# facebookresearch/multimodal

Measured on NVIDIA H100. Metric: image-text pairs/sec (CLIP ViT-B/16 contrastive pretrain step, bs=512/GPU), higher is better.
Workload: dtype bf16

## Files before the change

multimodal_b200/csrc/common.cuh:

```cuda
#pragma once
#include <cuda.h>
#include <cuda_bf16.h>
#include <cuda_runtime.h>
#include <stdint.h>
#include <stdio.h>

namespace mmb {

__device__ __forceinline__ uint32_t smem_u32(const void* p) {
  return static_cast<uint32_t>(__cvta_generic_to_shared(p));
}

__device__ __forceinline__ uint64_t global_timer_ns() {
  uint64_t t;
  asm volatile("mov.u64 %0, %%globaltimer;" : "=l"(t));
  return t;
}

#ifndef MMB_WATCHDOG_NS
#define MMB_WATCHDOG_NS 4000000000ull
#endif

__device__ __forceinline__ void mbar_init(uint64_t* bar, uint32_t count) {
  asm volatile("mbarrier.init.shared::cta.b64 [%0], %1;" ::"r"(smem_u32(bar)), "r"(count) : "memory");
}
__device__ __forceinline__ void fence_mbar_init() {
  asm volatile("fence.mbarrier_init.release.cluster;" ::: "memory");
}
__device__ __forceinline__ void fence_proxy_async_smem() {
  asm volatile("fence.proxy.async.shared::cta;" ::: "memory");
}
__device__ __forceinline__ void mbar_arrive_expect_tx(uint64_t* bar, uint32_t bytes) {
  asm volatile("mbarrier.arrive.expect_tx.shared::cta.b64 _, [%0], %1;" ::"r"(smem_u32(bar)), "r"(bytes)
               : "memory");
}
__device__ __forceinline__ void mbar_arrive(uint64_t* bar) {
  asm volatile("mbarrier.arrive.shared::cta.b64 _, [%0];" ::"r"(smem_u32(bar)) : "memory");
}
__device__ __forceinline__ void mbar_arrive_cluster(uint64_t* bar, uint32_t cta) {
  uint32_t remote;
  asm volatile("mapa.shared::cluster.u32 %0, %1, %2;" : "=r"(remote) : "r"(smem_u32(bar)), "r"(cta));
  asm volatile("mbarrier.arrive.shared::cluster.b64 _, [%0];" ::"r"(remote) : "memory");
}
__device__ __forceinline__ bool mbar_try_wait(uint64_t* bar, uint32_t parity) {
  uint32_t ok;
  asm volatile(
      "{\n\t.reg .pred p;\n\t"
      "mbarrier.try_wait.parity.shared::cta.b64 p, [%1], %2;\n\t"
      "selp.u32 %0, 1, 0, p;\n\t}"
      : "=r"(ok)
      : "r"(smem_u32(bar)), "r"(parity)
      : "memory");
  return ok != 0;
}
__device__ __forceinline__ void mbar_wait(uint64_t* bar, uint32_t parity) {
  if (mbar_try_wait(bar, parity)) return;
  uint32_t polls = 0;
  uint64_t t0 = 0;
  while (!mbar_try_wait(bar, parity)) {
#ifdef MMB_WAIT_NANOSLEEP
    __nanosleep(MMB_WAIT_NANOSLEEP);
#endif
    if ((++polls & 1023u) == 0) {
      const uint64_t now = global_timer_ns();
      if (t0 == 0) t0 = now;
      else if (now - t0 > MMB_WATCHDOG_NS) {
        printf("mmb watchdog: mbarrier wait timed out (block %d thread %d parity %u)\n", (int)blockIdx.x,
               (int)threadIdx.x, parity);
        __trap();
      }
    }
  }
}

__device__ __forceinline__ void mbar_wait_quiet(uint64_t* bar, uint32_t parity) {
  if (mbar_try_wait(bar, parity)) return;
  uint32_t polls = 0;
  uint64_t t0 = 0;
  while (!mbar_try_wait(bar, parity)) {
    if ((++polls & 1023u) == 0) {
      const uint64_t now = global_timer_ns();
      if (t0 == 0) t0 = now;
      else if (now - t0 > MMB_WATCHDOG_NS) __trap();
    }
  }
}

__device__ __forceinline__ void tma_prefetch_desc(const CUtensorMap* m) {
  asm volatile("prefetch.tensormap [%0];" ::"l"(reinterpret_cast<uint64_t>(m)) : "memory");
}
__device__ __forceinline__ void tma_prefetch_l2_2d(const CUtensorMap* m, int c0, int c1) {
  asm volatile("cp.async.bulk.prefetch.tensor.2d.L2.global.tile [%0, {%1, %2}];" ::"l"(reinterpret_cast<uint64_t>(m)),
               "r"(c0), "r"(c1)
               : "memory");
}
__device__ __forceinline__ void tma_load_2d(const CUtensorMap* m, uint64_t* bar, void* smem, int c0, int c1) {
  asm volatile(
      "cp.async.bulk.tensor.2d.shared::cluster.global.mbarrier::complete_tx::bytes [%0], [%1, {%3, %4}], [%2];"
      ::"r"(smem_u32(smem)), "l"(reinterpret_cast<uint64_t>(m)), "r"(smem_u32(bar)), "r"(c0), "r"(c1)
      : "memory");
}
__device__ __forceinline__ void tma_load_3d(const CUtensorMap* m, uint64_t* bar, void* smem, int c0, int c1,
                                            int c2) {
  asm volatile(
      "cp.async.bulk.tensor.3d.shared::cluster.global.mbarrier::complete_tx::bytes [%0], [%1, {%3, %4, %5}], [%2];"
      ::"r"(smem_u32(smem)), "l"(reinterpret_cast<uint64_t>(m)), "r"(smem_u32(bar)), "r"(c0), "r"(c1), "r"(c2)
      : "memory");
}
__device__ __forceinline__ void tma_store_2d(const CUtensorMap* m, const void* smem, int c0, int c1) {
  asm volatile("cp.async.bulk.tensor.2d.global.shared::cta.bulk_group [%0, {%2, %3}], [%1];" ::"l"(
                   reinterpret_cast<uint64_t>(m)),
               "r"(smem_u32(smem)), "r"(c0), "r"(c1)
               : "memory");
}
__device__ __forceinline__ void tma_store_3d(const CUtensorMap* m, const void* smem, int c0, int c1, int c2) {
  asm volatile("cp.async.bulk.tensor.3d.global.shared::cta.bulk_group [%0, {%2, %3, %4}], [%1];" ::"l"(
                   reinterpret_cast<uint64_t>(m)),
               "r"(smem_u32(smem)), "r"(c0), "r"(c1), "r"(c2)
               : "memory");
}
__device__ __forceinline__ void tma_reduce_add_2d(const CUtensorMap* m, const void* smem, int c0, int c1) {
  asm volatile("cp.reduce.async.bulk.tensor.2d.global.shared::cta.add.bulk_group [%0, {%2, %3}], [%1];" ::"l"(
                   reinterpret_cast<uint64_t>(m)),
               "r"(smem_u32(smem)), "r"(c0), "r"(c1)
               : "memory");
}
__device__ __forceinline__ void tma_store_commit() { asm volatile("cp.async.bulk.commit_group;" ::: "memory"); }
template <int N>
__device__ __forceinline__ void tma_store_wait_read() {
  asm volatile("cp.async.bulk.wait_group.read %0;" ::"n"(N) : "memory");
}
template <int N>
__device__ __forceinline__ void tma_store_wait_all() {
  asm volatile("cp.async.bulk.wait_group %0;" ::"n"(N) : "memory");
}

__device__ __forceinline__ uint32_t cluster_ctarank() {
  uint32_t r;
  asm volatile("mov.u32 %0, %%cluster_ctarank;" : "=r"(r));
  return r;
}
__device__ __forceinline__ void cluster_sync_all() {
  asm volatile("barrier.cluster.arrive.release.aligned;\n\tbarrier.cluster.wait.acquire.aligned;" ::: "memory");
}
__device__ __forceinline__ void tma_load_2d_multicast(const CUtensorMap* m, uint64_t* bar, void* smem, int c0, int c1,
                                                      uint16_t cta_mask) {
  asm volatile(
      "cp.async.bulk.tensor.2d.shared::cluster.global.mbarrier::complete_tx::bytes.multicast::cluster [%0], [%1, {%3, "
      "%4}], [%2], %5;" ::"r"(smem_u32(smem)),
      "l"(reinterpret_cast<uint64_t>(m)), "r"(smem_u32(bar)), "r"(c0), "r"(c1), "h"(cta_mask)
      : "memory");
}

__device__ __forceinline__ uint64_t make_smem_desc_sw128(uint32_t saddr, uint32_t lbo_bytes, uint32_t sbo_bytes) {
  uint64_t d = 0;
  d |= (uint64_t)((saddr & 0x3FFFFu) >> 4);
  d |= (uint64_t)((lbo_bytes >> 4) & 0x3FFFu) << 16;
  d |= (uint64_t)((sbo_bytes >> 4) & 0x3FFFu) << 32;
  d |= (uint64_t)1 << 62;
  return d;
}
__device__ __forceinline__ void wgmma_fence() { asm volatile("wgmma.fence.sync.aligned;" ::: "memory"); }
__device__ __forceinline__ void wgmma_commit() { asm volatile("wgmma.commit_group.sync.aligned;" ::: "memory"); }
template <int N>
__device__ __forceinline__ void wgmma_wait() {
  asm volatile("wgmma.wait_group.sync.aligned %0;" ::"n"(N) : "memory");
}
template <int TA, int TB>
__device__ __forceinline__ void wgmma_m64n256k16(float (&d)[128], uint64_t adesc, uint64_t bdesc, uint32_t accumulate) {
  asm volatile(
      "{\n\t.reg .pred p;\n\t"
      "setp.ne.b32 p, %130, 0;\n\t"
      "wgmma.mma_async.sync.aligned.m64n256k16.f32.bf16.bf16 "
      "{"
      "%0, %1, %2, %3, %4, %5, %6, %7, %8, %9, %10, %11, %12, %13, %14, %15, "
      "%16, %17, %18, %19, %20, %21, %22, %23, %24, %25, %26, %27, %28, %29, %30, %31, "
      "%32, %33, %34, %35, %36, %37, %38, %39, %40, %41, %42, %43, %44, %45, %46, %47, "
      "%48, %49, %50, %51, %52, %53, %54, %55, %56, %57, %58, %59, %60, %61, %62, %63, "
      "%64, %65, %66, %67, %68, %69, %70, %71, %72, %73, %74, %75, %76, %77, %78, %79, "
      "%80, %81, %82, %83, %84, %85, %86, %87, %88, %89, %90, %91, %92, %93, %94, %95, "
      "%96, %97, %98, %99, %100, %101, %102, %103, %104, %105, %106, %107, %108, %109, %110, %111, "
      "%112, %113, %114, %115, %116, %117, %118, %119, %120, %121, %122, %123, %124, %125, %126, %127"
      "}, %128, %129, p, 1, 1, %131, %132;\n\t}"
      : "+f"(d[0]), "+f"(d[1]), "+f"(d[2]), "+f"(d[3]), "+f"(d[4]), "+f"(d[5]), "+f"(d[6]), "+f"(d[7]),
        "+f"(d[8]), "+f"(d[9]), "+f"(d[10]), "+f"(d[11]), "+f"(d[12]), "+f"(d[13]), "+f"(d[14]), "+f"(d[15]),
        "+f"(d[16]), "+f"(d[17]), "+f"(d[18]), "+f"(d[19]), "+f"(d[20]), "+f"(d[21]), "+f"(d[22]), "+f"(d[23]),
        "+f"(d[24]), "+f"(d[25]), "+f"(d[26]), "+f"(d[27]), "+f"(d[28]), "+f"(d[29]), "+f"(d[30]), "+f"(d[31]),
        "+f"(d[32]), "+f"(d[33]), "+f"(d[34]), "+f"(d[35]), "+f"(d[36]), "+f"(d[37]), "+f"(d[38]), "+f"(d[39]),
        "+f"(d[40]), "+f"(d[41]), "+f"(d[42]), "+f"(d[43]), "+f"(d[44]), "+f"(d[45]), "+f"(d[46]), "+f"(d[47]),
        "+f"(d[48]), "+f"(d[49]), "+f"(d[50]), "+f"(d[51]), "+f"(d[52]), "+f"(d[53]), "+f"(d[54]), "+f"(d[55]),
        "+f"(d[56]), "+f"(d[57]), "+f"(d[58]), "+f"(d[59]), "+f"(d[60]), "+f"(d[61]), "+f"(d[62]), "+f"(d[63]),
        "+f"(d[64]), "+f"(d[65]), "+f"(d[66]), "+f"(d[67]), "+f"(d[68]), "+f"(d[69]), "+f"(d[70]), "+f"(d[71]),
        "+f"(d[72]), "+f"(d[73]), "+f"(d[74]), "+f"(d[75]), "+f"(d[76]), "+f"(d[77]), "+f"(d[78]), "+f"(d[79]),
        "+f"(d[80]), "+f"(d[81]), "+f"(d[82]), "+f"(d[83]), "+f"(d[84]), "+f"(d[85]), "+f"(d[86]), "+f"(d[87]),
        "+f"(d[88]), "+f"(d[89]), "+f"(d[90]), "+f"(d[91]), "+f"(d[92]), "+f"(d[93]), "+f"(d[94]), "+f"(d[95]),
        "+f"(d[96]), "+f"(d[97]), "+f"(d[98]), "+f"(d[99]), "+f"(d[100]), "+f"(d[101]), "+f"(d[102]), "+f"(d[103]),
        "+f"(d[104]), "+f"(d[105]), "+f"(d[106]), "+f"(d[107]), "+f"(d[108]), "+f"(d[109]), "+f"(d[110]), "+f"(d[111]),
        "+f"(d[112]), "+f"(d[113]), "+f"(d[114]), "+f"(d[115]), "+f"(d[116]), "+f"(d[117]), "+f"(d[118]), "+f"(d[119]),
        "+f"(d[120]), "+f"(d[121]), "+f"(d[122]), "+f"(d[123]), "+f"(d[124]), "+f"(d[125]), "+f"(d[126]), "+f"(d[127])
      : "l"(adesc), "l"(bdesc), "r"(accumulate), "n"(TA), "n"(TB));
}

template <int N>
__device__ __forceinline__ void setmaxnreg_dec() { asm volatile("setmaxnreg.dec.sync.aligned.u32 %0;" ::"n"(N)); }
template <int N>
__device__ __forceinline__ void setmaxnreg_inc() { asm volatile("setmaxnreg.inc.sync.aligned.u32 %0;" ::"n"(N)); }

__device__ __forceinline__ void ldsm_x4(uint32_t (&r)[4], uint32_t addr) {
  asm volatile("ldmatrix.sync.aligned.m8n8.x4.shared.b16 {%0,%1,%2,%3}, [%4];"
               : "=r"(r[0]), "=r"(r[1]), "=r"(r[2]), "=r"(r[3])
               : "r"(addr));
}
__device__ __forceinline__ void ldsm_x4_t(uint32_t (&r)[4], uint32_t addr) {
  asm volatile("ldmatrix.sync.aligned.m8n8.x4.trans.shared.b16 {%0,%1,%2,%3}, [%4];"
               : "=r"(r[0]), "=r"(r[1]), "=r"(r[2]), "=r"(r[3])
               : "r"(addr));
}
__device__ __forceinline__ void mma16816(float (&d)[4], const uint32_t (&a)[4], uint32_t b0, uint32_t b1) {
  asm volatile(
      "mma.sync.aligned.m16n8k16.row.col.f32.bf16.bf16.f32 {%0,%1,%2,%3}, {%4,%5,%6,%7}, {%8,%9}, {%0,%1,%2,%3};"
      : "+f"(d[0]), "+f"(d[1]), "+f"(d[2]), "+f"(d[3])
      : "r"(a[0]), "r"(a[1]), "r"(a[2]), "r"(a[3]), "r"(b0), "r"(b1));
}

__device__ __forceinline__ uint32_t pack_bf16x2(float lo, float hi) {
  __nv_bfloat162 v = __floats2bfloat162_rn(lo, hi);
  return *reinterpret_cast<uint32_t*>(&v);
}
__device__ __forceinline__ float bf16_lo(uint32_t v) { return __uint_as_float(v << 16); }
__device__ __forceinline__ float bf16_hi(uint32_t v) { return __uint_as_float(v & 0xFFFF0000u); }

__device__ __forceinline__ float ex2_approx(float x) {
  float y;
  asm("ex2.approx.ftz.f32 %0, %1;" : "=f"(y) : "f"(x));
  return y;
}
__device__ __forceinline__ float rcp_approx(float x) {
  float y;
  asm("rcp.approx.ftz.f32 %0, %1;" : "=f"(y) : "f"(x));
  return y;
}
__device__ __forceinline__ float fast_sigmoid(float z) {
  return rcp_approx(1.f + ex2_approx(-1.4426950408889634f * z));
}
__device__ __forceinline__ float tanh_approx(float x) {
  float y;
  asm("tanh.approx.f32 %0, %1;" : "=f"(y) : "f"(x));
  return y;
}
__device__ __forceinline__ float quick_gelu(float x) {
  const float t = tanh_approx(0.851f * x), h = 0.5f * x;
  return fmaf(h, t, h);
}
__device__ __forceinline__ float quick_gelu_grad(float x) {
  const float u = 0.851f * x;
  const float t = tanh_approx(u);
  return fmaf(0.5f, fmaf(u, fmaf(-t, t, 1.f), t), 0.5f);
}
__device__ __forceinline__ float gelu_erf(float x) { return 0.5f * x * (1.f + erff(x * 0.70710678118654752f)); }
__device__ __forceinline__ float gelu_erf_grad(float x) {
  return 0.5f * (1.f + erff(x * 0.70710678118654752f)) + x * 0.3989422804014327f * ex2_approx(-0.7213475204444817f * x * x);
}
template <int ACT>
__device__ __forceinline__ float act_fn(float x) { return ACT == 0 ? quick_gelu(x) : gelu_erf(x); }
template <int ACT>
__device__ __forceinline__ float act_grad(float x) { return ACT == 0 ? quick_gelu_grad(x) : gelu_erf_grad(x); }

}
```

multimodal_b200/csrc/gemm.cu:

```cuda
#include "common.cuh"
#include "mmb200_internal.h"
#include <stdlib.h>
#include <mutex>

namespace mmb {

constexpr int BLOCK_M = 128;
constexpr int BLOCK_N = 256;
constexpr int BLOCK_K = 64;
constexpr int WG_K = 16;
constexpr int STAGES = 4;
constexpr int A_BYTES = BLOCK_M * BLOCK_K * 2;
constexpr int B_BYTES = BLOCK_N * BLOCK_K * 2;
constexpr int GEMM_THREADS = 384;
constexpr int STG_BYTES = 64 * 128;
constexpr int EPI_SMEM = 4 * STG_BYTES;
constexpr int GEMM_SMEM_BYTES = 1024  + STAGES * (A_BYTES + B_BYTES) + EPI_SMEM + 256 ;
static_assert(GEMM_SMEM_BYTES <= 227 * 1024, "H100: at most 227 KB of shared memory per block");

struct GemmArgs {
  int M, N, K;
  int m_tiles, n_tiles, splits, kb_total, kb_per_split;
  float alpha;
  const float* bias;
  const __nv_bfloat16* aux;
  long long ld_aux;
  void* d0; void* d1;
  long long ldd0, ldd1;
  float* colsum_part;
  float* splitk_ws;
  int ws_rows;
  int accumulate;
  int f32_direct;
  const float* ce_log_scale;
  int ce_label0;
  const int* ce_labels;
  int ce_n_total;
  float ce_smoothing;
  float ce_gs;
  float ce_loss_weight;
  const float* ce_lse_row;
  const float* ce_row_w;
  const float* ce_lse_col;
  const float* ce_col_w;
  int ce_col_lo, ce_col_hi;
  float4* ce_part;
  int ce_part_ld, ce_part0;
  float* ce_xlabel;
};

__device__ __forceinline__ void wg_bar_sync(int cw) { asm volatile("bar.sync %0, 128;" ::"r"(2 + cw) : "memory"); }

template <bool A_MN, bool B_MN, int EPI, int ACT, bool CLU>
__global__ void __launch_bounds__(GEMM_THREADS, 1)
gemm_kernel(const __grid_constant__ CUtensorMap tmA, const __grid_constant__ CUtensorMap tmB,
            const __grid_constant__ CUtensorMap tmC0, const __grid_constant__ CUtensorMap tmC1, const GemmArgs p) {
  extern __shared__ uint8_t smem_raw[];
  uint8_t* smem = smem_raw + ((1024u - (smem_u32(smem_raw) & 1023u)) & 1023u);
  uint8_t* sA = smem;
  uint8_t* sB = smem + STAGES * A_BYTES;
  uint8_t* sStg = smem + STAGES * (A_BYTES + B_BYTES);
  uint64_t* full_bar = reinterpret_cast<uint64_t*>(sStg + EPI_SMEM);
  uint64_t* empty_bar = full_bar + STAGES;
  uint64_t* aux_bar = empty_bar + STAGES;
  constexpr int TILE_M = CLU ? 2 * BLOCK_M : BLOCK_M;
  const int wg = threadIdx.x >> 7;

  if (threadIdx.x == 0) {
    tma_prefetch_desc(&tmA);
    tma_prefetch_desc(&tmB);
    for (int i = 0; i < STAGES; ++i) {
      mbar_init(&full_bar[i], 1);
      mbar_init(&empty_bar[i], CLU ? 4 : 2);
    }
    for (int i = 0; i < 4; ++i) mbar_init(&aux_bar[i], 1);
    fence_mbar_init();
  }
  if (CLU) cluster_sync_all(); else __syncthreads();

#define MMB_TILE_SCHEDULE                                                      \
  const uint32_t rank = CLU ? cluster_ctarank() : 0u;                          \
  const int tiles_mn = p.m_tiles * p.n_tiles;                                  \
  const int total_tiles = tiles_mn * p.splits;                                 \
  const int tile_first = CLU ? (int)(blockIdx.x >> 1) : (int)blockIdx.x;       \
  const int tile_step = CLU ? (int)(gridDim.x >> 1) : (int)gridDim.x;

  if (wg == 0) {
    setmaxnreg_dec<40>();
    MMB_TILE_SCHEDULE
    if (threadIdx.x == 0) {
      int stage = 0;
      uint32_t phase = 0;
      for (int t = tile_first; t < total_tiles; t += tile_step) {
        const int split = t / tiles_mn;
        const int rem = t - split * tiles_mn;
        const int m_blk = rem / p.n_tiles, n_blk = rem - m_blk * p.n_tiles;
        const int kb0 = split * p.kb_per_split;
        const int kb1 = min(kb0 + p.kb_per_split, p.kb_total);
        const int m_row = m_blk * TILE_M + (int)rank * BLOCK_M;
        for (int kb = kb0; kb < kb1; ++kb) {
          mbar_wait_quiet(&empty_bar[stage], phase ^ 1);
          mbar_arrive_expect_tx(&full_bar[stage], A_BYTES + B_BYTES);
          uint8_t* a_dst = sA + stage * A_BYTES;
          uint8_t* b_dst = sB + stage * B_BYTES;
          if (!A_MN) {
            tma_load_2d(&tmA, &full_bar[stage], a_dst, kb * BLOCK_K, m_row);
          } else {
#pragma unroll
            for (int j = 0; j < BLOCK_M / 64; ++j)
              tma_load_2d(&tmA, &full_bar[stage], a_dst + j * (64 * BLOCK_K * 2), m_row + j * 64, kb * BLOCK_K);
          }
          const int n0 = n_blk * BLOCK_N;
          if (CLU) {
            const int h = (int)rank;
            if (!B_MN) {
              tma_load_2d_multicast(&tmB, &full_bar[stage], b_dst + h * 16384, kb * BLOCK_K, n0 + h * 128, 3);
            } else {
#pragma unroll
              for (int c = 2 * h; c < 2 * h + 2; ++c)
                tma_load_2d_multicast(&tmB, &full_bar[stage], b_dst + c * 8192, n0 + c * 64, kb * BLOCK_K, 3);
            }
          } else {
            if (!B_MN) {
              tma_load_2d(&tmB, &full_bar[stage], b_dst, kb * BLOCK_K, n0);
            } else {
#pragma unroll
              for (int c = 0; c < 4; ++c) tma_load_2d(&tmB, &full_bar[stage], b_dst + c * 8192, n0 + c * 64, kb * BLOCK_K);
            }
          }
          if (++stage == STAGES) { stage = 0; phase ^= 1; }
        }
      }
    }
  } else {
    setmaxnreg_inc<232>();
    MMB_TILE_SCHEDULE
    const int cw = wg - 1;
    const int wq = (threadIdx.x >> 5) & 3;
    const int lane = threadIdx.x & 31;
    const int tq = lane & 3;
    const int rl = wq * 16 + (lane >> 2);
    const bool elected = (threadIdx.x & 127) == 0;
    uint8_t* stg = sStg + cw * 2 * STG_BYTES;
    constexpr uint32_t A_KSTEP = A_MN ? (WG_K / 8) * 1024 : WG_K * 2;
    constexpr uint32_t B_KSTEP = B_MN ? (WG_K / 8) * 1024 : WG_K * 2;
    constexpr uint32_t B_LBO = B_MN ? 64 * BLOCK_K * 2 : 16;
    int stage = 0;
    uint32_t phase = 0;
    uint32_t stg_next = 0;
    uint32_t aux_phase = 0;
    float acc[128];
    for (int t = tile_first; t < total_tiles; t += tile_step) {
      const int split = t / tiles_mn;
      const int rem = t - split * tiles_mn;
      const int m_blk = rem / p.n_tiles, n_blk = rem - m_blk * p.n_tiles;
      const int kb0 = split * p.kb_per_split;
      const int kb1 = min(kb0 + p.kb_per_split, p.kb_total);
      const int row0 = m_blk * TILE_M + (int)rank * BLOCK_M + cw * 64;
      const int col0 = n_blk * BLOCK_N;
      if (EPI == EPI_BF16_DACT && elected) {
        tma_store_wait_read<0>();
#pragma unroll
        for (int b = 0; b < 2; ++b)
          if (col0 + 64 * b < p.N) {
            mbar_arrive_expect_tx(&aux_bar[2 * cw + b], STG_BYTES);
            tma_load_2d(&tmC1, &aux_bar[2 * cw + b], stg + b * STG_BYTES, col0 + 64 * b, row0);
          }
      }
      int prev_stage = -1;
      for (int kb = kb0; kb < kb1; ++kb) {
        mbar_wait_quiet(&full_bar[stage], phase);
        const uint64_t adesc = make_smem_desc_sw128(smem_u32(sA + stage * A_BYTES + cw * 8192), 16, 1024);
        const uint64_t bdesc = make_smem_desc_sw128(smem_u32(sB + stage * B_BYTES), B_LBO, 1024);
        wgmma_fence();
#pragma unroll
        for (int k = 0; k < BLOCK_K / WG_K; ++k)
          wgmma_m64n256k16<A_MN ? 1 : 0, B_MN ? 1 : 0>(acc, adesc + (uint64_t)((k * A_KSTEP) >> 4),
                                                      bdesc + (uint64_t)((k * B_KSTEP) >> 4), (kb > kb0 || k > 0) ? 1u : 0u);
        wgmma_commit();
        wgmma_wait<1>();
        if (prev_stage >= 0 && threadIdx.x % 128 == 0) {
          mbar_arrive(&empty_bar[prev_stage]);
          if (CLU) mbar_arrive_cluster(&empty_bar[prev_stage], rank ^ 1u);
        }
        prev_stage = stage;
        if (++stage == STAGES) { stage = 0; phase ^= 1; }
      }
      wgmma_wait<0>();
      if (prev_stage >= 0 && threadIdx.x % 128 == 0) {
        mbar_arrive(&empty_bar[prev_stage]);
        if (CLU) mbar_arrive_cluster(&empty_bar[prev_stage], rank ^ 1u);
      }

      const int r[2] = {row0 + rl, row0 + rl + 8};
      const int nq = col0 + 2 * tq;
      const int n_left = p.N - nq;
      const bool add_bias = (p.bias != nullptr) && (split == 0);
      if (EPI == EPI_CE_STATS) {
        const float T = __expf(__ldg(p.ce_log_scale));
        const float T2 = T * 1.4426950408889634f;
#pragma unroll
        for (int h = 0; h < 2; ++h) {
          if (col0 + 128 * h >= p.N) continue;
#pragma unroll
          for (int i = 0; i < 2; ++i) {
            const int lab = p.ce_labels ? __ldg(p.ce_labels + min(r[i], p.M - 1)) : p.ce_label0 + r[i];
            const int lab_off = r[i] < p.M ? lab - nq : -1;
            float gm = -INFINITY;
#pragma unroll
            for (int j = 16 * h; j < 16 * h + 16; ++j)
#pragma unroll
              for (int e = 0; e < 2; ++e)
                if (8 * j + e < n_left) gm = fmaxf(gm, acc[4 * j + 2 * i + e]);
            float m2 = gm * T2, se = 0.f, sex = 0.f, sx = 0.f;
            if (gm > -INFINITY) {
#pragma unroll
              for (int j = 16 * h; j < 16 * h + 16; ++j)
#pragma unroll
                for (int e = 0; e < 2; ++e) {
                  if (8 * j + e < n_left) {
                    const float a = acc[4 * j + 2 * i + e];
                    const float x = a * T;
                    const float pe = ex2_approx(fmaf(a, T2, -m2));
                    se += pe; sex = fmaf(pe, x, sex); sx += x;
                    if (8 * j + e == lab_off) p.ce_xlabel[r[i]] = x;
                  }
                }
            }
#pragma unroll
            for (int o = 1; o <= 2; o <<= 1) {
              const float mo = __shfl_xor_sync(0xffffffffu, m2, o);
              const float seo = __shfl_xor_sync(0xffffffffu, se, o);
              const float sexo = __shfl_xor_sync(0xffffffffu, sex, o);
              const float sxo = __shfl_xor_sync(0xffffffffu, sx, o);
              const float mn = fmaxf(m2, mo);
              const float f = (m2 == -INFINITY) ? 0.f : ex2_approx(m2 - mn);
              const float fo = (mo == -INFINITY) ? 0.f : ex2_approx(mo - mn);
              se = se * f + seo * fo; sex = sex * f + sexo * fo; sx += sxo; m2 = mn;
            }
            if (tq == 0 && r[i] < p.M)
              p.ce_part[(long long)r[i] * p.ce_part_ld + p.ce_part0 + 2 * n_blk + h] =
                  make_float4(m2 * 0.6931471805599453f, se, sex, sx);
          }
        }
      } else if (EPI == EPI_F32) {
        if (p.f32_direct) {
          float* D = reinterpret_cast<float*>(p.d0);
#pragma unroll
          for (int j = 0; j < 32; ++j) {
            const int n = nq + 8 * j;
            if (n >= p.N) continue;
            float b0 = 0.f, b1 = 0.f;
            if (add_bias) { b0 = __ldg(p.bias + n); b1 = __ldg(p.bias + n + 1); }
#pragma unroll
            for (int i = 0; i < 2; ++i) {
              if (r[i] >= p.M) continue;
              const float v0 = fmaf(acc[4 * j + 2 * i], p.alpha, b0), v1 = fmaf(acc[4 * j + 2 * i + 1], p.alpha, b1);
              float* dst = D + (long long)r[i] * p.ldd0 + n;
              if (p.accumulate) { dst[0] += v0; dst[1] += v1; }
              else              { dst[0] = v0; dst[1] = v1; }
            }
          }
        } else {
#pragma unroll
          for (int q = 0; q < 8; ++q) {
            if (col0 + 32 * q >= p.N) continue;
            uint8_t* buf = stg + (stg_next & 1u) * STG_BYTES;
            if (elected) tma_store_wait_read<1>();
            wg_bar_sync(cw);
#pragma unroll
            for (int jj = 0; jj < 4; ++jj) {
              const int j = 4 * q + jj;
              const int n = nq + 8 * j;
              float b0 = 0.f, b1 = 0.f;
              if (add_bias && n < p.N) { b0 = __ldg(p.bias + n); b1 = __ldg(p.bias + n + 1); }
#pragma unroll
              for (int i = 0; i < 2; ++i) {
                const int rr = rl + 8 * i;
                float2* sp = reinterpret_cast<float2*>(buf + rr * 128 + (((2 * jj + (tq >> 1)) ^ (rr & 7)) << 4) + 8 * (tq & 1));
                *sp = make_float2(fmaf(acc[4 * j + 2 * i], p.alpha, b0), fmaf(acc[4 * j + 2 * i + 1], p.alpha, b1));
              }
            }
            fence_proxy_async_smem();
            wg_bar_sync(cw);
            if (elected) {
              if (p.splitk_ws)       tma_store_2d(&tmC0, buf, col0 + 32 * q, split * p.ws_rows + row0);
              else if (p.accumulate) tma_reduce_add_2d(&tmC0, buf, col0 + 32 * q, row0);
              else                   tma_store_2d(&tmC0, buf, col0 + 32 * q, row0);
              tma_store_commit();
            }
            ++stg_next;
          }
        }
      } else {
        float ce_T = 0.f, ce_T2 = 0.f, ce_eps_n = 0.f, ce_gcT = 0.f;
        float ce_lse2[2] = {0.f, 0.f}, ce_gsT[2] = {0.f, 0.f};
        if (EPI == EPI_CE_GRAD) {
          ce_T = __expf(__ldg(p.ce_log_scale));
          ce_T2 = ce_T * 1.4426950408889634f;
          ce_gcT = ce_T * p.ce_gs;
          ce_eps_n = p.ce_smoothing / (float)p.ce_n_total;
#pragma unroll
          for (int i = 0; i < 2; ++i) {
            const int gr = min(r[i], p.M - 1);
            ce_lse2[i] = __ldg(p.ce_lse_row + gr) * 1.4426950408889634f;
            ce_gsT[i] = ce_T * (p.ce_row_w ? p.ce_loss_weight * __ldg(p.ce_row_w + gr) : p.ce_gs);
          }
        }
        const bool do_colsum = (EPI == EPI_BF16 || EPI == EPI_BF16_DACT) && p.colsum_part != nullptr;
        float cs_keep[4][2];
        constexpr int PASSES = EPI == EPI_BF16_ACT ? 2 : 1;
#pragma unroll
        for (int ps = 0; ps < PASSES; ++ps) {
#pragma unroll
          for (int q = 0; q < 4; ++q) {
            cs_keep[q][0] = cs_keep[q][1] = 0.f;
            if (col0 + 64 * q >= p.N) continue;
            const uint32_t b = EPI == EPI_BF16_DACT ? (uint32_t)(q & 1) : (stg_next & 1u);
            uint8_t* buf = stg + b * STG_BYTES;
            if (EPI == EPI_BF16_DACT) {
              mbar_wait_quiet(&aux_bar[2 * cw + b], (aux_phase >> b) & 1u);
              aux_phase ^= 1u << b;
            } else {
              if (elected) tma_store_wait_read<1>();
              wg_bar_sync(cw);
            }
#pragma unroll
            for (int jj = 0; jj < 8; ++jj) {
              const int j = 8 * q + jj;
              const int n = nq + 8 * j;
              const bool col_ok = n < p.N;
              float b0 = 0.f, b1 = 0.f;
              if (add_bias && col_ok) { b0 = __ldg(p.bias + n); b1 = __ldg(p.bias + n + 1); }
              float cs0 = 0.f, cs1 = 0.f;
#pragma unroll
              for (int i = 0; i < 2; ++i) {
                const int rr = rl + 8 * i;
                uint32_t* sp = reinterpret_cast<uint32_t*>(buf + rr * 128 + ((jj ^ (rr & 7)) << 4) + 4 * tq);
                float f0, f1;
                if (EPI == EPI_CE_GRAD) {
                  float f[2];
#pragma unroll
                  for (int e = 0; e < 2; ++e) {
                    const int c = n + e;
                    const float a = acc[4 * j + 2 * i + e];
                    const float tt = ((c == p.ce_label0 + r[i]) ? (1.f - p.ce_smoothing) : 0.f) + ce_eps_n;
                    float gsum = ce_gsT[i] * (ex2_approx(fmaf(a, ce_T2, -ce_lse2[i])) - tt);
                    if (p.ce_lse_col != nullptr && c >= p.ce_col_lo && c < p.ce_col_hi && c < p.N) {
                      const float wc = p.ce_col_w ? p.ce_loss_weight * ce_T * __ldg(p.ce_col_w + c) : ce_gcT;
                      if (wc != 0.f) gsum += wc * (ex2_approx(fmaf(a, ce_T2, -__ldg(p.ce_lse_col + c) * 1.4426950408889634f)) - tt);
                    }
                    f[e] = gsum;
                  }
                  f0 = f[0]; f1 = f[1];
                } else {
                  f0 = fmaf(acc[4 * j + 2 * i], p.alpha, b0);
                  f1 = fmaf(acc[4 * j + 2 * i + 1], p.alpha, b1);
                }
                if (EPI == EPI_BF16_DACT) {
                  const uint32_t av = *sp;
                  f0 *= act_grad<ACT>(bf16_lo(av));
                  f1 *= act_grad<ACT>(bf16_hi(av));
                }
                uint32_t o = pack_bf16x2(f0, f1);
                if (EPI == EPI_BF16_ACT && ps == 1) o = pack_bf16x2(act_fn<ACT>(bf16_lo(o)), act_fn<ACT>(bf16_hi(o)));
                *sp = o;
                if (do_colsum && col_ok && r[i] < p.M) { cs0 += bf16_lo(o); cs1 += bf16_hi(o); }
              }
              if (do_colsum) {
#pragma unroll
                for (int o = 4; o <= 16; o <<= 1) {
                  cs0 += __shfl_xor_sync(0xffffffffu, cs0, o);
                  cs1 += __shfl_xor_sync(0xffffffffu, cs1, o);
                }
                if ((lane >> 2) == jj) { cs_keep[q][0] = cs0; cs_keep[q][1] = cs1; }
              }
            }
            fence_proxy_async_smem();
            wg_bar_sync(cw);
            if (elected) {
              tma_store_2d(EPI == EPI_BF16_ACT && ps == 1 ? &tmC1 : &tmC0, buf, col0 + 64 * q, row0);
              tma_store_commit();
              if (EPI == EPI_BF16_DACT && q + 2 < 4 && col0 + 64 * (q + 2) < p.N) {
                tma_store_wait_read<0>();
                mbar_arrive_expect_tx(&aux_bar[2 * cw + b], STG_BYTES);
                tma_load_2d(&tmC1, &aux_bar[2 * cw + b], buf, col0 + 64 * (q + 2), row0);
              }
            }
            if (EPI != EPI_BF16_DACT) ++stg_next;
          }
        }
        if (do_colsum) {
          if (elected) tma_store_wait_read<0>();
          wg_bar_sync(cw);
          float* sCol = reinterpret_cast<float*>(stg) + wq * BLOCK_N;
#pragma unroll
          for (int q = 0; q < 4; ++q) {
            const int c = 8 * (8 * q + (lane >> 2)) + 2 * tq;
            sCol[c] = cs_keep[q][0];
            sCol[c + 1] = cs_keep[q][1];
          }
          asm volatile("bar.sync 1, 256;" ::: "memory");
          const int ct = threadIdx.x - 128, blk_row = m_blk * TILE_M + (int)rank * BLOCK_M;
          if (blk_row < p.M && col0 + ct < p.N) {
            const float* all = reinterpret_cast<const float*>(sStg);
            float s = 0.f;
#pragma unroll
            for (int w = 0; w < 8; ++w) s += all[(w >> 2) * (2 * STG_BYTES / 4) + (w & 3) * BLOCK_N + ct];
            p.colsum_part[(long long)(blk_row / BLOCK_M) * p.N + col0 + ct] = s;
          }
          fence_proxy_async_smem();
          asm volatile("bar.sync 1, 256;" ::: "memory");
        }
      }
    }
    if (elected) tma_store_wait_all<0>();
  }
  if (CLU) cluster_sync_all();
}
#undef MMB_TILE_SCHEDULE

typedef CUresult (*PFN_encodeTiled)(CUtensorMap*, CUtensorMapDataType, cuuint32_t, void*, const cuuint64_t*,
                                    const cuuint64_t*, const cuuint32_t*, const cuuint32_t*, CUtensorMapInterleave,
                                    CUtensorMapSwizzle, CUtensorMapL2promotion, CUtensorMapFloatOOBfill);

static PFN_encodeTiled get_encode_fn() {
  static PFN_encodeTiled fn = nullptr;
  if (!fn) {
    void* p = nullptr;
    cudaDriverEntryPointQueryResult qres;
    if (cudaGetDriverEntryPoint("cuTensorMapEncodeTiled", &p, cudaEnableDefault, &qres) != cudaSuccess || !p)
      return nullptr;
    fn = reinterpret_cast<PFN_encodeTiled>(p);
  }
  return fn;
}

struct TmapKey {
  const void* ptr; uint64_t inner, outer, pitch; uint32_t box_inner, box_outer, kind;
  bool operator==(const TmapKey& o) const {
    return ptr == o.ptr && inner == o.inner && outer == o.outer && pitch == o.pitch && box_inner == o.box_inner &&
           box_outer == o.box_outer && kind == o.kind;
  }
};
struct TmapSlot { TmapKey key; CUtensorMap map; bool valid; };
constexpr int TMAP_CACHE_SLOTS = 4096;
static TmapSlot* g_tmap_cache = nullptr;
static std::mutex g_tmap_mu;

int make_tmap_2d(CUtensorMap* out, const void* ptr, int elem_bytes, bool is_f32, uint64_t inner, uint64_t outer,
                 uint64_t pitch_bytes, uint32_t box_inner, uint32_t box_outer) {
  PFN_encodeTiled enc = get_encode_fn();
  if (!enc) return MMB_ERR_DRIVER;
  if ((reinterpret_cast<uintptr_t>(ptr) & 15) || (pitch_bytes & 15) || box_inner * elem_bytes != 128) return MMB_ERR_ARG;
  const TmapKey key{ptr, inner, outer, pitch_bytes, box_inner, box_outer, (uint32_t)(is_f32 ? 1 : 0)};
  uint64_t hsh = reinterpret_cast<uintptr_t>(ptr) * 0x9E3779B97F4A7C15ull;
  hsh ^= (inner * 0xC2B2AE3D27D4EB4Full) ^ (outer * 0x165667B19E3779F9ull) ^ (pitch_bytes << 17) ^
         ((uint64_t)box_outer << 40) ^ ((uint64_t)box_inner << 52) ^ key.kind;
  const int slot = (int)((hsh >> 20) % TMAP_CACHE_SLOTS);
  {
    std::lock_guard<std::mutex> lk(g_tmap_mu);
    if (!g_tmap_cache) g_tmap_cache = new TmapSlot[TMAP_CACHE_SLOTS]();
    if (g_tmap_cache[slot].valid && g_tmap_cache[slot].key == key) {
      *out = g_tmap_cache[slot].map;
      return MMB_OK;
    }
  }
  cuuint64_t gdim[2] = {inner, outer};
  cuuint64_t gstr[1] = {pitch_bytes};
  cuuint32_t box[2] = {box_inner, box_outer};
  cuuint32_t estr[2] = {1, 1};
  CUresult r = enc(out, is_f32 ? CU_TENSOR_MAP_DATA_TYPE_FLOAT32 : CU_TENSOR_MAP_DATA_TYPE_BFLOAT16, 2,
                   const_cast<void*>(ptr), gdim, gstr, box, estr, CU_TENSOR_MAP_INTERLEAVE_NONE,
                   CU_TENSOR_MAP_SWIZZLE_128B, CU_TENSOR_MAP_L2_PROMOTION_L2_256B, CU_TENSOR_MAP_FLOAT_OOB_FILL_NONE);
  if (r != CUDA_SUCCESS) return MMB_ERR_DRIVER;
  {
    std::lock_guard<std::mutex> lk(g_tmap_mu);
    g_tmap_cache[slot].key = key;
    g_tmap_cache[slot].map = *out;
    g_tmap_cache[slot].valid = true;
  }
  return MMB_OK;
}

int make_tmap_3d_bf16(CUtensorMap* out, const void* ptr, uint64_t inner, uint64_t dim1, uint64_t dim2, uint64_t pitch1,
                      uint64_t pitch2, uint32_t box_inner, uint32_t box1) {
  PFN_encodeTiled enc = get_encode_fn();
  if (!enc) return MMB_ERR_DRIVER;
  if ((reinterpret_cast<uintptr_t>(ptr) & 15) || (pitch1 & 15) || (pitch2 & 15) || box_inner * 2 != 128) return MMB_ERR_ARG;
  cuuint64_t gdim[3] = {inner, dim1, dim2};
  cuuint64_t gstr[2] = {pitch1, pitch2};
  cuuint32_t box[3] = {box_inner, box1, 1};
  cuuint32_t estr[3] = {1, 1, 1};
  CUresult r = enc(out, CU_TENSOR_MAP_DATA_TYPE_BFLOAT16, 3, const_cast<void*>(ptr), gdim, gstr, box, estr,
                   CU_TENSOR_MAP_INTERLEAVE_NONE, CU_TENSOR_MAP_SWIZZLE_128B, CU_TENSOR_MAP_L2_PROMOTION_L2_256B,
                   CU_TENSOR_MAP_FLOAT_OOB_FILL_NONE);
  return r == CUDA_SUCCESS ? MMB_OK : MMB_ERR_DRIVER;
}

static int g_num_sms = 0;
int num_sms() {
  if (!g_num_sms) {
    int dev = 0;
    cudaGetDevice(&dev);
    cudaDeviceGetAttribute(&g_num_sms, cudaDevAttrMultiProcessorCount, dev);
  }
  return g_num_sms;
}

template <bool A_MN, bool B_MN, int EPI, int ACT, bool CLU>
static int launch_impl(const CUtensorMap& tA, const CUtensorMap& tB, const CUtensorMap& tC0, const CUtensorMap& tC1,
                       const GemmArgs& args, cudaStream_t stream) {
  auto kfn = gemm_kernel<A_MN, B_MN, EPI, ACT, CLU>;
  static bool attr_set = false;
  if (!attr_set) {
    cudaError_t e = cudaFuncSetAttribute(kfn, cudaFuncAttributeMaxDynamicSharedMemorySize, GEMM_SMEM_BYTES);
    if (e != cudaSuccess) return (int)e;
    attr_set = true;
  }
  const int total = args.m_tiles * args.n_tiles * args.splits;
  cudaLaunchConfig_t cfg{};
  cudaLaunchAttribute attr[1];
  if (CLU) {
    const int clusters = total < num_sms() / 2 ? total : num_sms() / 2;
    cfg.gridDim = dim3(2 * clusters);
    attr[0].id = cudaLaunchAttributeClusterDimension;
    attr[0].val.clusterDim.x = 2; attr[0].val.clusterDim.y = 1; attr[0].val.clusterDim.z = 1;
    cfg.attrs = attr; cfg.numAttrs = 1;
  } else {
    cfg.gridDim = dim3(total < num_sms() ? total : num_sms());
  }
  cfg.blockDim = dim3(GEMM_THREADS);
  cfg.dynamicSmemBytes = GEMM_SMEM_BYTES;
  cfg.stream = stream;
  return (int)cudaLaunchKernelEx(&cfg, kfn, tA, tB, tC0, tC1, args);
}

}

using namespace mmb;

static int g_force_cta2 = -1;
extern "C" int mmb_gemm_set_mode(int cta2, int epilogue_warps) {
  if (cta2 < -1 || cta2 > 1 || (epilogue_warps != 0 && epilogue_warps != 8)) return MMB_ERR_ARG;
  g_force_cta2 = cta2;
  return MMB_OK;
}

__global__ void splitk_reduce_kernel(const float* __restrict__ ws, int S, int M, int ws_rows, int N, float* __restrict__ D,
                                     long long ldd, int accumulate) {
  const int n = (blockIdx.x * blockDim.x + threadIdx.x) * 4;
  if (n >= N) return;
  for (int m = blockIdx.y; m < M; m += gridDim.y) {
    float* dst = D + (long long)m * ldd + n;
    float4 acc = accumulate ? make_float4(dst[0], dst[1], dst[2], dst[3]) : make_float4(0.f, 0.f, 0.f, 0.f);
    for (int s = 0; s < S; ++s) {
      const float4 v = *reinterpret_cast<const float4*>(ws + ((long long)s * ws_rows + m) * N + n);
      acc.x += v.x; acc.y += v.y; acc.z += v.z; acc.w += v.w;
    }
    dst[0] = acc.x; dst[1] = acc.y; dst[2] = acc.z; dst[3] = acc.w;
  }
}

static int gemm_launch(int a_mn_major, int b_mn_major, int epilogue, int act, bool cta2, const CUtensorMap& tA,
                       const CUtensorMap& tB, const CUtensorMap& tC0, const CUtensorMap& tC1, const GemmArgs& g,
                       cudaStream_t stream);

static int gemm_dispatch(const void* A, long long lda, int a_mn_major, const void* B, long long ldb, int b_mn_major,
                         void* D0, long long ldd0, void* D1, long long ldd1, int M, int N, int K, int epilogue, int act,
                         float alpha, const float* bias, const void* aux, long long ld_aux, int splits, int accumulate,
                         float* colsum, const GemmArgs* ce, void* stream_) {
  cudaStream_t stream = reinterpret_cast<cudaStream_t>(stream_);
  if (M <= 0 || N <= 0 || K <= 0) return MMB_ERR_ARG;
  if ((epilogue == EPI_CE_STATS || epilogue == EPI_CE_GRAD) && (!ce || a_mn_major || b_mn_major)) return MMB_ERR_ARG;
  if ((lda & 7) || (ldb & 7)) return MMB_ERR_ARG;
  if (epilogue != EPI_CE_STATS && (epilogue == EPI_F32 ? (N & 3) : (N & 7))) return MMB_ERR_ARG;
  const long long big_tiles = (long long)((M + 2 * BLOCK_M - 1) / (2 * BLOCK_M)) * ((N + BLOCK_N - 1) / BLOCK_N);
  const bool cta2 = g_force_cta2 == 1 ||
                    (g_force_cta2 == -1 && M >= 512 && big_tiles * (splits < 1 ? 1 : splits) >= num_sms() / 2);
  GemmArgs g{};
  if (ce) g = *ce;
  g.M = M; g.N = N; g.K = K;
  g.m_tiles = cta2 ? (M + 2 * BLOCK_M - 1) / (2 * BLOCK_M) : (M + BLOCK_M - 1) / BLOCK_M;
  g.n_tiles = (N + BLOCK_N - 1) / BLOCK_N;
  g.kb_total = (K + BLOCK_K - 1) / BLOCK_K;
  if (splits < 1) splits = 1;
  if (splits > g.kb_total) splits = g.kb_total;
  if (epilogue != EPI_F32) splits = 1;
  g.kb_per_split = (g.kb_total + splits - 1) / splits;
  g.splits = (g.kb_total + g.kb_per_split - 1) / g.kb_per_split;
  g.alpha = alpha;
  g.bias = bias;
  g.aux = reinterpret_cast<const __nv_bfloat16*>(aux);
  g.ld_aux = ld_aux;
  g.d0 = D0; g.d1 = D1; g.ldd0 = ldd0; g.ldd1 = ldd1;
  g.accumulate = accumulate ? 1 : 0;
  if (colsum && (epilogue == EPI_F32 || epilogue == EPI_BF16_ACT)) return MMB_ERR_ARG;
  const int col_blocks = (M + BLOCK_M - 1) / BLOCK_M;
  if (colsum) {
    g.colsum_part = static_cast<float*>(scratch(SCR_GEMM_COLSUM, (size_t)col_blocks * N * sizeof(float), stream));
    if (!g.colsum_part) return (int)cudaErrorMemoryAllocation;
  }
  if (epilogue == EPI_F32 && g.splits > 1) {
    g.ws_rows = g.m_tiles * (cta2 ? 2 * BLOCK_M : BLOCK_M);
    g.splitk_ws = static_cast<float*>(scratch(SCR_GEMM_SPLITK, (size_t)g.splits * g.ws_rows * N * sizeof(float), stream));
    if (!g.splitk_ws) return (int)cudaErrorMemoryAllocation;
  }

  CUtensorMap tA, tB;
  int rc;
  if (!a_mn_major) rc = make_tmap_2d(&tA, A, 2, false, K, M, lda * 2, 64, BLOCK_M);
  else             rc = make_tmap_2d(&tA, A, 2, false, M, K, lda * 2, 64, BLOCK_K);
  if (rc) return rc;
  if (!b_mn_major) rc = make_tmap_2d(&tB, B, 2, false, K, N, ldb * 2, 64, cta2 ? BLOCK_N / 2 : BLOCK_N);
  else             rc = make_tmap_2d(&tB, B, 2, false, N, K, ldb * 2, 64, BLOCK_K);
  if (rc) return rc;
  CUtensorMap tC0 = tA, tC1 = tA;
  if (epilogue == EPI_F32) {
    if (ldd0 & 3) return MMB_ERR_ARG;
    if (g.splitk_ws) {
      rc = make_tmap_2d(&tC0, g.splitk_ws, 4, true, N, (uint64_t)g.splits * g.ws_rows, (uint64_t)N * 4, 32, 64);
    } else if ((reinterpret_cast<uintptr_t>(D0) & 15) == 0 && (ldd0 & 3) == 0) {
      rc = make_tmap_2d(&tC0, D0, 4, true, N, M, ldd0 * 4, 32, 64);
    } else {
      g.f32_direct = 1;
    }
    if (rc) return rc;
  } else if (epilogue != EPI_CE_STATS) {
    if ((ldd0 & 7) || (reinterpret_cast<uintptr_t>(D0) & 15)) return MMB_ERR_ARG;
    if (epilogue == EPI_BF16_ACT && (!D1 || (ldd1 & 7) || (reinterpret_cast<uintptr_t>(D1) & 15))) return MMB_ERR_ARG;
    if (epilogue == EPI_BF16_DACT && (!aux || (ld_aux & 7) || (reinterpret_cast<uintptr_t>(aux) & 15))) return MMB_ERR_ARG;
    rc = make_tmap_2d(&tC0, D0, 2, false, N, M, ldd0 * 2, 64, 64);
    if (!rc && epilogue == EPI_BF16_ACT) rc = make_tmap_2d(&tC1, D1, 2, false, N, M, ldd1 * 2, 64, 64);
    if (!rc && epilogue == EPI_BF16_DACT) rc = make_tmap_2d(&tC1, aux, 2, false, N, M, ld_aux * 2, 64, 64);
    if (rc) return rc;
  }

  int rc_launch = gemm_launch(a_mn_major, b_mn_major, epilogue, act, cta2, tA, tB, tC0, tC1, g, stream);
  if (rc_launch) return rc_launch;
  if (g.splitk_ws) {
    splitk_reduce_kernel<<<dim3((N / 4 + 127) / 128, M < 65535 ? M : 65535), 128, 0, stream>>>(
        g.splitk_ws, g.splits, M, g.ws_rows, N, reinterpret_cast<float*>(D0), ldd0, g.accumulate);
    rc_launch = (int)cudaGetLastError();
    if (rc_launch) return rc_launch;
  }
  if (colsum) return reduce_partials(g.colsum_part, col_blocks, N, N, colsum, 1, stream);
  return MMB_OK;
}

static int gemm_launch(int a_mn_major, int b_mn_major, int epilogue, int act, bool cta2, const CUtensorMap& tA,
                       const CUtensorMap& tB, const CUtensorMap& tC0, const CUtensorMap& tC1, const GemmArgs& g,
                       cudaStream_t stream) {
  const int am = a_mn_major ? 1 : 0, bm = b_mn_major ? 1 : 0;
  if (epilogue == EPI_CE_STATS)
    return cta2 ? launch_impl<false, false, EPI_CE_STATS, 0, true>(tA, tB, tC0, tC1, g, stream)
                : launch_impl<false, false, EPI_CE_STATS, 0, false>(tA, tB, tC0, tC1, g, stream);
  if (epilogue == EPI_CE_GRAD)
    return cta2 ? launch_impl<false, false, EPI_CE_GRAD, 0, true>(tA, tB, tC0, tC1, g, stream)
                : launch_impl<false, false, EPI_CE_GRAD, 0, false>(tA, tB, tC0, tC1, g, stream);
#define MMB_CASE(AM, BM, E, AC)                                                                                   \
  if (am == AM && bm == BM && epilogue == E && (AC < 0 || act == AC))                                             \
    return cta2 ? launch_impl<(AM != 0), (BM != 0), E, (AC < 0 ? 0 : AC), true>(tA, tB, tC0, tC1, g, stream)                \
                : launch_impl<(AM != 0), (BM != 0), E, (AC < 0 ? 0 : AC), false>(tA, tB, tC0, tC1, g, stream);
  MMB_CASE(0, 0, EPI_BF16, -1)
  MMB_CASE(0, 0, EPI_BF16_ACT, ACT_QUICK_GELU)
  MMB_CASE(0, 0, EPI_BF16_ACT, ACT_GELU_ERF)
  MMB_CASE(0, 0, EPI_F32, -1)
  MMB_CASE(0, 1, EPI_BF16, -1)
  MMB_CASE(0, 1, EPI_BF16_DACT, ACT_QUICK_GELU)
  MMB_CASE(0, 1, EPI_BF16_DACT, ACT_GELU_ERF)
  MMB_CASE(0, 1, EPI_F32, -1)
  MMB_CASE(1, 1, EPI_F32, -1)
  MMB_CASE(1, 0, EPI_F32, -1)
#undef MMB_CASE
  return MMB_ERR_UNSUPPORTED;
}
extern "C" int mmb_gemm_bf16(const void* A, long long lda, int a_mn_major, const void* B, long long ldb,
                             int b_mn_major, void* D0, long long ldd0, void* D1, long long ldd1, int M, int N, int K,
                             int epilogue, int act, float alpha, const float* bias, const void* aux,
                             long long ld_aux, int splits, int accumulate, float* colsum, void* stream_) {
  if (epilogue < EPI_BF16 || epilogue > EPI_F32) return MMB_ERR_ARG;
  return gemm_dispatch(A, lda, a_mn_major, B, ldb, b_mn_major, D0, ldd0, D1, ldd1, M, N, K, epilogue, act, alpha, bias,
                       aux, ld_aux, splits, accumulate, colsum, nullptr, stream_);
}

extern "C" int mmb_gemm_ce_num_parts(int N) { return N <= 0 ? 0 : (N + 127) / 128; }

static int gemm_ce_stats_impl(const void* A, long long lda, const void* B, long long ldb, int M, int N, int K,
                              const float* log_scale, int label0, const int* labels, void* part, int part_ld, int part0,
                              float* xlabel, void* stream) {
  if (!log_scale || !part || !xlabel || part_ld <= 0 || part0 < 0 || part0 + mmb_gemm_ce_num_parts(N) > part_ld ||
      (reinterpret_cast<uintptr_t>(part) & 15))
    return MMB_ERR_ARG;
  GemmArgs ce{};
  ce.ce_log_scale = log_scale; ce.ce_label0 = label0; ce.ce_labels = labels;
  ce.ce_part = reinterpret_cast<float4*>(part); ce.ce_part_ld = part_ld; ce.ce_part0 = part0; ce.ce_xlabel = xlabel;
  return gemm_dispatch(A, lda, 0, B, ldb, 0, nullptr, 0, nullptr, 0, M, N, K, EPI_CE_STATS, 0, 1.f, nullptr, nullptr, 0, 1, 0,
                       nullptr, &ce, stream);
}

extern "C" int mmb_gemm_ce_stats(const void* A, long long lda, const void* B, long long ldb, int M, int N, int K,
                                 const float* log_scale, int label0, void* part, int part_ld, int part0, float* xlabel,
                                 void* stream) {
  return gemm_ce_stats_impl(A, lda, B, ldb, M, N, K, log_scale, label0, nullptr, part, part_ld, part0, xlabel, stream);
}
extern "C" int mmb_gemm_ce_stats_labels(const void* A, long long lda, const void* B, long long ldb, int M, int N, int K,
                                        const float* log_scale, const int* labels, void* part, int part_ld, int part0,
                                        float* xlabel, void* stream) {
  if (!labels) return MMB_ERR_ARG;
  return gemm_ce_stats_impl(A, lda, B, ldb, M, N, K, log_scale, 0, labels, part, part_ld, part0, xlabel, stream);
}

extern "C" int mmb_gemm_ce_grad(const void* A, long long lda, const void* B, long long ldb, int M, int N, int K,
                                const float* log_scale, int label0, int n_total, int rows_total, float smoothing,
                                float loss_weight, const float* lse_row, const float* row_w, const float* lse_col,
                                const float* col_w, int col_lo, int col_hi, void* dsims_bf16, long long ldd,
                                void* stream) {
  if (!log_scale || !lse_row || !dsims_bf16 || n_total <= 0 || rows_total <= 0) return MMB_ERR_ARG;
  GemmArgs ce{};
  ce.ce_log_scale = log_scale; ce.ce_label0 = label0; ce.ce_n_total = n_total; ce.ce_smoothing = smoothing;
  ce.ce_loss_weight = loss_weight; ce.ce_gs = loss_weight / (float)rows_total;
  ce.ce_lse_row = lse_row; ce.ce_row_w = row_w; ce.ce_lse_col = lse_col; ce.ce_col_w = col_w;
  ce.ce_col_lo = col_lo; ce.ce_col_hi = col_hi;
  return gemm_dispatch(A, lda, 0, B, ldb, 0, dsims_bf16, ldd, nullptr, 0, M, N, K, EPI_CE_GRAD, 0, 1.f, nullptr, nullptr, 0, 1,
                       0, nullptr, &ce, stream);
}
```

Measured before the change: 3114.

## Rework GEMM epilogue: smem colsum, batched aux prefetch, bias L1 prefetch

Column sums in the bf16 epilogue are now computed by reading the staged tile back from shared memory after the TMA store is issued, replacing per-element accumulation plus warp shuffles in the hot write loop. For the DACT epilogue, activation-gradient inputs are loaded from the staging buffer in groups of four ahead of use, and bias is disabled for the DACT and CE_GRAD paths. A bias L1 prefetch is issued at tile start. The smem colsum pass adds extra shared-memory reads and, on DACT with colsum, an extra barrier before reusing the buffer.

After: 3202, median of 6. +2.8%, better.

```diff
diff --git a/multimodal_b200/csrc/common.cuh b/multimodal_b200/csrc/common.cuh
--- a/multimodal_b200/csrc/common.cuh
+++ b/multimodal_b200/csrc/common.cuh
@@ -88,6 +88,9 @@
 
 __device__ __forceinline__ void tma_prefetch_desc(const CUtensorMap* m) {
   asm volatile("prefetch.tensormap [%0];" ::"l"(reinterpret_cast<uint64_t>(m)) : "memory");
+}
+__device__ __forceinline__ void prefetch_l1(const void* p) {
+  asm volatile("prefetch.global.L1 [%0];" ::"l"(reinterpret_cast<uint64_t>(p)));
 }
 __device__ __forceinline__ void tma_prefetch_l2_2d(const CUtensorMap* m, int c0, int c1) {
   asm volatile("cp.async.bulk.prefetch.tensor.2d.L2.global.tile [%0, {%1, %2}];" ::"l"(reinterpret_cast<uint64_t>(m)),
diff --git a/multimodal_b200/csrc/gemm.cu b/multimodal_b200/csrc/gemm.cu
--- a/multimodal_b200/csrc/gemm.cu
+++ b/multimodal_b200/csrc/gemm.cu
@@ -158,6 +158,8 @@
       const int kb1 = min(kb0 + p.kb_per_split, p.kb_total);
       const int row0 = m_blk * TILE_M + (int)rank * BLOCK_M + cw * 64;
       const int col0 = n_blk * BLOCK_N;
+      if (p.bias != nullptr && split == 0 && wq == 0 && lane < 8 && col0 + 32 * lane < p.N)
+        prefetch_l1(p.bias + col0 + 32 * lane);
       if (EPI == EPI_BF16_DACT && elected) {
         tma_store_wait_read<0>();
 #pragma unroll
@@ -195,7 +197,7 @@
       const int r[2] = {row0 + rl, row0 + rl + 8};
       const int nq = col0 + 2 * tq;
       const int n_left = p.N - nq;
-      const bool add_bias = (p.bias != nullptr) && (split == 0);
+      const bool add_bias = EPI != EPI_BF16_DACT && EPI != EPI_CE_GRAD && (p.bias != nullptr) && (split == 0);
       if (EPI == EPI_CE_STATS) {
         const float T = __expf(__ldg(p.ce_log_scale));
         const float T2 = T * 1.4426950408889634f;
@@ -325,14 +327,24 @@
               if (elected) tma_store_wait_read<1>();
               wg_bar_sync(cw);
             }
+            constexpr int PRE = 4;
+            uint32_t pre[PRE][2];
 #pragma unroll
             for (int jj = 0; jj < 8; ++jj) {
               const int j = 8 * q + jj;
               const int n = nq + 8 * j;
               const bool col_ok = n < p.N;
+              if (EPI == EPI_BF16_DACT && jj % PRE == 0) {
+#pragma unroll
+                for (int u = 0; u < PRE; ++u)
+#pragma unroll
+                  for (int i = 0; i < 2; ++i) {
+                    const int rr = rl + 8 * i;
+                    pre[u][i] = *reinterpret_cast<const uint32_t*>(buf + rr * 128 + (((jj + u) ^ (rr & 7)) << 4) + 4 * tq);
+                  }
+              }
               float b0 = 0.f, b1 = 0.f;
               if (add_bias && col_ok) { b0 = __ldg(p.bias + n); b1 = __ldg(p.bias + n + 1); }
-              float cs0 = 0.f, cs1 = 0.f;
 #pragma unroll
               for (int i = 0; i < 2; ++i) {
                 const int rr = rl + 8 * i;
@@ -358,22 +370,13 @@
                   f1 = fmaf(acc[4 * j + 2 * i + 1], p.alpha, b1);
                 }
                 if (EPI == EPI_BF16_DACT) {
-                  const uint32_t av = *sp;
+                  const uint32_t av = pre[jj % PRE][i];
                   f0 *= act_grad<ACT>(bf16_lo(av));
                   f1 *= act_grad<ACT>(bf16_hi(av));
                 }
                 uint32_t o = pack_bf16x2(f0, f1);
                 if (EPI == EPI_BF16_ACT && ps == 1) o = pack_bf16x2(act_fn<ACT>(bf16_lo(o)), act_fn<ACT>(bf16_hi(o)));
                 *sp = o;
-                if (do_colsum && col_ok && r[i] < p.M) { cs0 += bf16_lo(o); cs1 += bf16_hi(o); }
-              }
-              if (do_colsum) {
-#pragma unroll
-                for (int o = 4; o <= 16; o <<= 1) {
-                  cs0 += __shfl_xor_sync(0xffffffffu, cs0, o);
-                  cs1 += __shfl_xor_sync(0xffffffffu, cs1, o);
-                }
-                if ((lane >> 2) == jj) { cs_keep[q][0] = cs0; cs_keep[q][1] = cs1; }
               }
             }
             fence_proxy_async_smem();
@@ -381,7 +384,49 @@
             if (elected) {
               tma_store_2d(EPI == EPI_BF16_ACT && ps == 1 ? &tmC1 : &tmC0, buf, col0 + 64 * q, row0);
               tma_store_commit();
-              if (EPI == EPI_BF16_DACT && q + 2 < 4 && col0 + 64 * (q + 2) < p.N) {
+            }
+            if (do_colsum) {
+              float sb0[2];
+#pragma unroll 1
+              for (int h = 0; h < 2; ++h) {
+                float sa[2][2];
+#pragma unroll
+                for (int pq = 0; pq < 2; ++pq) {
+                  float sg[2][2];
+#pragma unroll
+                  for (int u = 0; u < 2; ++u) {
+                    const int g = 4 * h + 2 * pq + u;
+                    sg[u][0] = sg[u][1] = 0.f;
+#pragma unroll
+                    for (int i = 0; i < 2; ++i) {
+                      const int rr = wq * 16 + g + 8 * i;
+                      if (row0 + rr < p.M) {
+                        const uint32_t w = *reinterpret_cast<const uint32_t*>(buf + rr * 128 + (((lane >> 2) ^ g) << 4) +
+                                                                              4 * (lane & 3));
+                        sg[u][0] += bf16_lo(w);
+                        sg[u][1] += bf16_hi(w);
+                      }
+                    }
+                  }
+                  sa[pq][0] = sg[0][0] + sg[1][0];
+                  sa[pq][1] = sg[0][1] + sg[1][1];
+                }
+                const float sb[2] = {sa[0][0] + sa[1][0], sa[0][1] + sa[1][1]};
+                if (h == 0) {
+                  sb0[0] = sb[0];
+                  sb0[1] = sb[1];
+                } else {
+                  cs_keep[q][0] = sb0[0] + sb[0];
+                  cs_keep[q][1] = sb0[1] + sb[1];
+                }
+              }
+            }
+            if (EPI == EPI_BF16_DACT && q + 2 < 4 && col0 + 64 * (q + 2) < p.N) {
+              if (do_colsum) {
+                fence_proxy_async_smem();
+                wg_bar_sync(cw);
+              }
+              if (elected) {
                 tma_store_wait_read<0>();
                 mbar_arrive_expect_tx(&aux_bar[2 * cw + b], STG_BYTES);
                 tma_load_2d(&tmC1, &aux_bar[2 * cw + b], buf, col0 + 64 * (q + 2), row0);
@@ -596,6 +641,7 @@
   g.d0 = D0; g.d1 = D1; g.ldd0 = ldd0; g.ldd1 = ldd1;
   g.accumulate = accumulate ? 1 : 0;
   if (colsum && (epilogue == EPI_F32 || epilogue == EPI_BF16_ACT)) return MMB_ERR_ARG;
+  if (bias && epilogue == EPI_BF16_DACT) return MMB_ERR_ARG;
   const int col_blocks = (M + BLOCK_M - 1) / BLOCK_M;
   if (colsum) {
     g.colsum_part = static_cast<float*>(scratch(SCR_GEMM_COLSUM, (size_t)col_blocks * N * sizeof(float), stream));
```
